# xiaohong-huang/RTK-Visual-Inertial-Navigation

Measured on AMD Instinct MI355X. Metric: gauss_newton_iterations_per_sec, higher is better.
Workload: dtype f64; 1 GPU; BASELINE cfg4: batch of 512 independent cfg3 windows (20 keyframes, 300 features, 3000 observations, 19 IMU factors, 10 satellites x 20 epochs carrier-phase+pseudorange, gauge prior) over the job, 8 dogleg iterations per solve; windows=512, windows_rank0=512

## Files before the change

rtk_visual_inertial_navigation_amd/csrc/swf_dev.h:

```cpp
#pragma once
#include <hip/hip_runtime.h>
#include <stdint.h>
#include "../../include/swf_types.h"

#define SWF_WAVE 64

struct WinRec {
    int x_base, x_n;
    int blk_base, n_blk;
    int loc_base, n_loc, n_e, n_red;
    long long S_base;
    long long Lt_base;
    int proj0, proj1;
    int lm0, lm1;
    int fr_base, nF;
    long long P_base;
    int gf0, gf1;
    int cl0, cl1;
    int pair0, pair1;
    int fsb0, fsb1;
    int tail_dim;
    int n_pose_blk;
    int lmb0, lmb1;
    int pch0, pch1;
// ... 9 lines not shown
    int status, iter, need_lin, reuse, eval_cand, lin_fail, invalid_run, nsucc, nunsucc;
    int chol_fail;
};

enum { GF_IMU = 1, GF_CP = 2, GF_PR = 3, GF_DOP = 4, GF_SP = 5, GF_PRIOR = 6, GF_SPR = 7, GF_SCP = 8, GF_FIX = 9, GF_IDP = 10,
       GF_PROJX = 11 };
struct GFac {
    int type, win, nres, nslot;
    int slot0;
    int roff;
    int data;
    int clique;
    int jld;
    int pad;
};

struct Clique {
    int win;
    int e_loc, d_e;
    int d_f;
    int fac0, fac1;
    int mem0, mem1;
    long long C_off;
    int v_off;
    int e_off;
    int is_static;
    int n_rows;
    int j_off, r_off;
    int pad0, pad1;
};
// ... 59 lines not shown
    const int* sch_c0; const int* sch_rec;
    const int* sch_km;
    const unsigned long long* lm_fmask;
    int n_fr;
    const int* fr_obs0; const int* fr_obs;
    const int* fr_red;
    int n_gf;
    const GFac* gf;
    const int* s_x; const int* s_loc; const int* s_ls; const int* s_joff; const int* s_ccol;
    double* g_r; double* g_J; double* g_cost; double* g_aux;
    const double* imu_pre; const double* cp_dat; const double* pr_dat; const double* dop_dat; const double* sp_w;
    const double* gx_dat;
    int n_imu; const int* imu_gf;
    int n_idp; const int* idp_gf;
    int n_sc;  const int* sc_gf;
    int n_prior; const int* prior_gf;
    int n_pch; const int* pch_q; const int* pch_r0; const int* prior_nch;
    double* pr_cpart; double* pr_apart;
    const int* prior_dim; const long long* prior_Joff; const int* prior_roff; const int* prior_x0off;
    const double* prior_J; const double* prior_r0; const double* prior_x0;
    const double* prior_Jt;
    const int* prior_colloc;
    const int* prior_colcc;
    const int* s_pcol; const int* s_pxo;
    int n_cl;
    const Clique* cl;
    const int* cl_fac; const int* cl_frow;
    const int* cm_loc; const int* cm_ls; const int* cm_col;
    double* C; double* cv_graw; double* cv_dgraw; double* cv_cs; double* cE;
    const int* cv_loc;
// ... 262 lines not shown
```

rtk_visual_inertial_navigation_amd/csrc/swf_engine.hip:

```cpp
#include <hip/hip_runtime.h>
#include <algorithm>
#include <array>
#include <chrono>
#include <cmath>
#include <cstdio>
#include <cstdlib>
#include <cstring>
#include <map>
#include <string>
#include <memory>
#include <thread>
#include <vector>
#include "../../include/swf_solver.h"
#include "swf_kernels2.h"
#include "swf_kernels3.h"
#include "swf_kernels4.h"
#include "swf_lambda.h"
#include "swf_features.h"

static thread_local std::string g_err;
static int fail(int code, const std::string& msg) { g_err = msg; return code; }
#define HIPCHK(x) do { hipError_t e_ = (x); if (e_ != hipSuccess) return fail(SWF_E_NODEVICE, std::string(#x) + ": " + hipGetErrorString(e_)); } while (0)

extern "C" const char* swf_last_error(void) { return g_err.c_str(); }
// ... 191 lines not shown
        if (aux) { (void)hipStreamSynchronize(aux); handle_cache().give(aux); }
        for (auto& e : ev_fork) handle_cache().give(e, false);
    }
    WinState* ws_primary = nullptr; WinState* ws_alt = nullptr; WinState* ws_alt2 = nullptr;
    bool no_decide_fuse = false;
    bool no_step_fuse = false;
    int n_pch_split = 0;
    bool no_spec = false;
    bool no_comp_fuse = false;
    bool lat_fuse = false;
    bool rr4_has15 = false, rr4_has16 = false;
    int rr_nmax = 256;
    bool L_full = false;
    int asm_programs = 0;
    int ls_qpb = 1, ls_var = 0, ls_kms = 8; bool ls_folded = false, s_direct = false;
    int timing = 0;
    swf_timing last{};
    std::vector<hipEvent_t> ev;
    std::vector<int> ev_kind;
    int ev_used = 0;
    int64_t jac_bytes = 0, proj_bytes = 0, chol_flops = 0, lm_schur_flops = 0, lm_schur_flops_sym = 0, lm_schur_mfma = 0;
    int last_mode = -1;
};

namespace {
struct Build {
    std::vector<WinRec> win;
    std::vector<int> blk_xoff, blk_loc, blk_gs, loc2x;
    std::vector<unsigned char> x_var;
    std::vector<int> p_win, p_xpose, p_xex, p_xlm, p_lpose, p_llm, p_fr, p_lm;
// ... 552 lines not shown
    std::vector<HostWin> hw(n);
    for (int i = 0; i < n; i++) {
        int rc = build_window(B, windows[i], i, hw[i]);
        if (rc != SWF_OK) return rc;
    }
    if (B.n_x > 0x7fffffffLL || B.n_loc > 0x7fffffffLL) return fail(SWF_E_UNSUPPORTED, "batch too large for 32-bit offsets");
    swf_batch* b = new swf_batch();
    b->device = current_device();
    b->stream = (hipStream_t)stream;
    { int dev = 0; hipDeviceProp_t pr; if (hipGetDevice(&dev) == hipSuccess && hipGetDeviceProperties(&pr, dev) == hipSuccess && pr.multiProcessorCount > 0) b->n_cu = pr.multiProcessorCount; }
    b->D.rr_nmax = b->rr_nmax;
    b->no_comp_fuse = getenv("SWF_NO_COMP_FUSE") != nullptr;
    b->no_spec = getenv("SWF_NO_SPEC_EVAL") != nullptr;
    b->no_step_fuse = getenv("SWF_NO_STEP_FUSE") != nullptr;
    b->no_decide_fuse = getenv("SWF_NO_DECIDE_FUSE") != nullptr;
    b->lat_fuse = n * 8 <= b->n_cu && !getenv("SWF_NO_LAT_FUSE");
    if ((n * 16 <= b->n_cu && !b->lat_fuse) || (2 * n >= b->n_cu && n <= b->n_cu)) {
        bool ok = (b->aux = handle_cache().stream()) != nullptr;
        for (int i = 0; i < 3 && ok; i++) ok = (b->ev_fork[i] = handle_cache().event(false)) != nullptr;
        if (!ok) { handle_cache().give(b->aux); b->aux = nullptr; }
    }
    b->win = B.win; b->hw = hw; b->max_tiles = B.max_tiles; b->max_prior_dim = B.max_prior_dim; b->jac_bytes = B.jac_bytes;
    b->proj_bytes = (int64_t)312 * (int64_t)B.p_win.size();
    for (size_t l = 0; l + 1 < B.lm_obs0.size() + 1 && l < B.lm_win.size(); l++) {
        int64_t k = (l + 1 < B.lm_obs0.size() ? B.lm_obs0[l + 1] : (int)B.p_win.size()) - B.lm_obs0[l];
        b->lm_schur_flops += 216 * k * k + 108 * k;
        b->lm_schur_flops_sym += 108 * k * (k - 1) + 162 * k;
    }
    for (auto& W : B.win) { b->chol_flops += (int64_t)W.n_red * W.n_red * W.n_red / 3; b->max_red = std::max(b->max_red, W.n_red); b->min_red = std::min(b->min_red, W.n_red); if (W.n_red > 224 && W.n_red <= 240) b->rr4_has15 = true; if (W.n_red > 240 && W.n_red <= 256) b->rr4_has16 = true; }
    DevBatch& D = b->D;
// ... 48 lines not shown
    PUT(p_lpose, B.p_lpose); PUT(p_llm, B.p_llm); PUT(p_fr, B.p_fr); PUT(p_lm, B.p_lm); PUT(p_uv, B.p_uv);
    D.n_lm = (int)B.lm_win.size();
    B.lm_obs0.push_back(D.n_proj);
    PUT(lm_win, B.lm_win); PUT(lm_obs0, B.lm_obs0); PUT(lm_loc, B.lm_loc); PUT(lm_col, B.lm_col); PUT(lm_fmask, B.lm_fmask);
    {
        const int force = getenv("SWF_LS_VARIANT") ? atoi(getenv("SWF_LS_VARIANT")) : 0;
        const int force_qpb = getenv("SWF_LS_QPB") ? atoi(getenv("SWF_LS_QPB")) : 0;
        int qpb = 1;
        while (qpb < GEMM_SPLIT && (long long)n * GEMM_SPLIT / (2 * qpb) >= 2LL * b->n_cu) qpb *= 2;
        if (2LL * n >= b->n_cu) qpb = GEMM_SPLIT;
        if (force_qpb >= 1 && force_qpb <= GEMM_SPLIT && (force_qpb & (force_qpb - 1)) == 0) qpb = force_qpb;
        b->ls_qpb = qpb;
        b->ls_var = (b->max_tiles <= 10 && force < 1) ? 0 : (b->max_tiles <= 36 && force < 2) ? 1 : (b->max_tiles <= 136 && force < 3) ? 2 : 3;
        b->ls_folded = qpb == GEMM_SPLIT && b->ls_var <= 1;
        b->s_direct = b->ls_folded;
    }
    {
        const int TW = b->ls_var <= 1 ? 2 : 1;
        const int NCW = b->ls_var <= 1 ? 8 : 12, TPW = b->ls_var == 0 ? 2 : b->ls_var == 1 ? 5 : 6;
        const int n_launch = std::max(1, (b->max_tiles + NCW * TPW - 1) / (NCW * TPW));
        b->ls_kms = n_launch * NCW;
        std::vector<int> c0, rec, km;
        std::vector<std::vector<unsigned>> task_tiles;
        for (auto& W : B.win) {
            const int m = 6 * W.nF, nt = (m + 15) / 16, ntl = nt * (nt + 1) / 2;
            auto tile_rows = [&](unsigned long long fm) {
                unsigned t = 0;
                for (int f = 0; f < W.nF && f < 64; f++) if ((fm >> f) & 1ULL) { t |= 1u << ((6 * f) / 16); t |= 1u << ((6 * f + 5) / 16); }
                return t;
            };
// ... 58 lines not shown
            int* r = rec.data() + (size_t)8 * k;
            r[0] = B.fsb_win[(size_t)k]; r[1] = B.fsb_obs0[(size_t)k]; r[2] = B.fsb_obs0[(size_t)k + 1] - B.fsb_obs0[(size_t)k];
            r[3] = B.fsb_foff0[(size_t)k]; r[4] = B.fsb_out0[(size_t)k]; r[5] = B.win[(size_t)r[0]].nF;
        }
        PUT(fsb_rec, rec);
    }
    PUT(fsb_perm, B.fsb_perm); PUT(fsb_foff, B.fsb_foff);
    rc |= P.zeros((size_t)B.fs_tot * FS_VAL, &D.fs_part);
    rc |= P.zeros((size_t)std::max<long long>(B.n_loc, 1), &D.jsc);
    D.n_gf = (int)B.gf.size();
    PUT(gf, B.gf);
    PUT(s_x, B.s_x); PUT(s_loc, B.s_loc); PUT(s_ls, B.s_ls); PUT(s_joff, B.s_joff); PUT(s_ccol, B.s_ccol);
    PUT(imu_pre, B.imu_pre); PUT(cp_dat, B.cp_dat); PUT(pr_dat, B.pr_dat); PUT(dop_dat, B.dop_dat); PUT(sp_w, B.sp_w); PUT(gx_dat, B.gx_dat);
    D.n_imu = (int)B.imu_gf.size(); D.n_sc = (int)B.sc_gf.size(); D.n_prior = (int)B.prior_gf.size();
    PUT(imu_gf, B.imu_gf); PUT(sc_gf, B.sc_gf); PUT(prior_gf, B.prior_gf); D.n_idp = (int)B.idp_gf.size(); PUT(idp_gf, B.idp_gf);
    PUT(prior_dim, B.prior_dim); PUT(prior_Joff, B.prior_Joff); PUT(prior_roff, B.prior_roff); PUT(prior_x0off, B.prior_x0off);
    {
        std::vector<double> Jt(B.prior_J.size());
        for (size_t k = 0; k < B.prior_dim.size(); k++) {
            const size_t n = (size_t)B.prior_dim[k]; const double* J = B.prior_J.data() + B.prior_Joff[k]; double* T = Jt.data() + B.prior_Joff[k];
            for (size_t r = 0; r < n; r++) for (size_t c = 0; c < n; c++) T[c * n + r] = J[r * n + c];
        }
        PUT(prior_Jt, Jt);
        std::vector<int> cl(B.prior_r0.size(), -1), cc(B.prior_r0.size(), -1), pcol(B.s_ls.size(), 0), pxo(B.s_ls.size(), 0);
        for (const GFac& G : B.gf) {
            if (G.type != GF_PRIOR) continue;
            int col = 0, xo = 0;
            for (int t = 0; t < G.nslot; t++) {
                int l = B.s_ls[G.slot0 + t], lo = B.s_loc[G.slot0 + t], mc = B.s_ccol[G.slot0 + t];
                pcol[G.slot0 + t] = col; pxo[G.slot0 + t] = xo;
// ... 479 lines not shown
            if (imu_fused) hipLaunchKernelGGL((k_eval_ps<true, true, true>), dim3(S.e[3]), dim3(256), 0, st, D, S);
            else hipLaunchKernelGGL((k_eval_ps<true, true>), dim3(S.e[2]), dim3(256), 0, st, D, S);
        }
        if (D.n_idp) hipLaunchKernelGGL(k_eval_idp<true>, GRID(D.n_idp, 128), dim3(128), 0, st, D);
        if (D.n_prior && b->max_prior_dim > PRIOR_LDS_DIM) { Bracket t(*this, SWF_K_EVAL_PRIOR); hipLaunchKernelGGL(k_eval_prior<true>, dim3(D.n_pch), dim3(256), (2 * b->max_prior_dim + 16) * sizeof(double), st, D); }
        if (fork) (void)hipEventRecord(b->ev_fork[1], st);
        if (D.n_imu && !imu_fused) { Bracket t(*this, SWF_K_EVAL_IMU, sa); hipLaunchKernelGGL(k_eval_imu<true>, GRID(D.n_imu, IMU_FPB), dim3(IMU_FPB * IMU_LPF), 0, sa, D); }
    }
    void lin_elim(int write_S) {
        DevBatch& D = b->D;
        bool clq_fused = false;
        if (comp_fused) {
            Bracket t(*this, SWF_K_CLIQUE_ELIM);
            if (D.n_clc[3]) {
                hipLaunchKernelGGL(k_clique_big2, dim3(D.n_clc[3] + D.n_clc[2]), dim3(CB_NT), 0, st, D, O);
                if (D.n_clc[4]) hipLaunchKernelGGL(k_clique_tall, dim3(D.n_clc[4]), dim3(256), 0, st, D, O);
            } else if (D.n_clc[4] + D.n_clc[2]) hipLaunchKernelGGL(k_clique_tall2, dim3(D.n_clc[4] + D.n_clc[2]), dim3(256), 0, st, D, O);
        } else if (D.n_lm) {
            Bracket t(*this, write_S ? SWF_K_LM_SCHUR : SWF_K_LM_ELIM);
            lm_qpb = b->ls_qpb; lm_folded = b->ls_folded;
            if (!write_S) {
                dim3 grid(D.n_win, GEMM_SPLIT / lm_qpb);
                hipLaunchKernelGGL((k_lm_schur<8, 2, 2, 80, false>), grid, dim3(256), 0, st, D, O, lm_qpb, 0, 0, 0);
            } else {
                const int crow = D.n_win > 0 ? (D.n_clc[2] + D.n_win - 1) / D.n_win : 0;
                clq_fused = clq_fuse_ok();
                lm_launch(0, st, clq_fused ? crow : 0);
                lm_next = ls_tiles_per_launch();
            }
        }
        {
            hipStream_t sa = b->aux ? b->aux : st;
            if (b->aux) (void)hipStreamWaitEvent(b->aux, b->ev_fork[1], 0);
            auto cstream = [&](int cls) { return (b->aux && !b->clc_imu[cls]) ? st : sa; };
            if (comp_fused) {
                for (; lm_next < b->max_tiles; lm_next += ls_tiles_per_launch()) { Bracket t(*this, SWF_K_LM_SCHUR, sa); lm_launch(lm_next, sa); }
            } else {
            if (D.n_clc[1]) { Bracket t(*this, SWF_K_CLIQUE_ELIM, cstream(1)); hipLaunchKernelGGL((k_clique_elim<32, 48, 9, 1>), dim3(D.n_clc[1]), dim3(64), 0, cstream(1), D, O); }
            if (D.n_clc[0]) { Bracket t(*this, SWF_K_CLIQUE_ELIM, cstream(0)); hipLaunchKernelGGL((k_clique_elim<48, 32, 1, 0>), dim3(D.n_clc[0]), dim3(64), 0, cstream(0), D, O); }
            if (D.n_clc[2] && !clq_fused) {
                Bracket t(*this, SWF_K_CLIQUE_ELIM, cstream(2));
                if (b->lat_fuse) hipLaunchKernelGGL(k_clique_elim4, dim3(D.n_clc[2]), dim3(256), 0, cstream(2), D, O);
                else hipLaunchKernelGGL((k_clique_elim<64, 64, 9, 2>), dim3(D.n_clc[2]), dim3(64), 0, cstream(2), D, O);
            }
            if (D.n_clc[3]) { Bracket t(*this, SWF_K_CLIQUE_ELIM, cstream(3)); hipLaunchKernelGGL(k_clique_big, dim3(D.n_clc[3]), dim3(CB_NT), 0, cstream(3), D, O); }
            if (D.n_clc[4]) { Bracket t(*this, SWF_K_CLIQUE_ELIM, cstream(4)); hipLaunchKernelGGL(k_clique_tall, dim3(D.n_clc[4]), dim3(256), 0, cstream(4), D, O); }
            if (write_S && D.n_lm) {
                for (; lm_next < b->max_tiles; lm_next += ls_tiles_per_launch()) { Bracket t(*this, SWF_K_LM_SCHUR, sa); lm_launch(lm_next, sa); }
            }
            }
            if (b->aux) (void)hipEventRecord(b->ev_fork[2], b->aux);
        }
        if (b->n_pch_split) hipLaunchKernelGGL(k_prior_graw, dim3(D.n_pch), dim3(256), 0, st, D);
        if (b->aux) (void)hipStreamWaitEvent(st, b->ev_fork[2], 0);
        if (D.n_pd) {
            Bracket t(*this, SWF_K_ASSEMBLE);
            const int nbS = write_S ? nb((size_t)D.as_max_ne, 256) : 0, nbV = nb((size_t)D.as_max_nv, 256);
            hipLaunchKernelGGL(k_assemble_flat, dim3(nbS + nbV, D.n_win), dim3(256), 0, st, D, O, write_S, nbS);
        }
    }
    void reduced() {
// ... 871 lines not shown
```

rtk_visual_inertial_navigation_amd/csrc/swf_kernels.h:

```cpp
#pragma once
#include "swf_dev.h"

struct DevOpt {
    int max_iter, step_mode, strategy, jacobi;
    double r0, max_r, min_r, min_rel_dec, ftol, gtol, ptol, min_mu, max_mu, mu_inc, min_diag, max_diag;
};



__device__ __forceinline__ double damp_diag(const DevOpt& O, double d, double* jsc_slot, bool first) {
    if (!O.jacobi) return clampd(d, O.min_diag, O.max_diag);
    double q;
    if (first) { double r = 1.0 + sqrt(d > 0.0 ? d : 0.0); q = r * r; *jsc_slot = q; }
    else q = *jsc_slot;
    return clampd(d / q, O.min_diag, O.max_diag) * q;
}

template <bool JAC> __device__ __forceinline__ bool eval_gate(const DevBatch& B, const WinState& s) { return B.spec == 2 ? true : (JAC && !B.spec) ? s.need_lin != 0 : s.eval_cand != 0; }
template <bool JAC> __device__ __forceinline__ const double* eval_src(const DevBatch& B) { return (JAC && !B.spec) ? B.x : B.xc; }

#define CLIGHT_D 299792458.0
#define OMGE_D 7.2921151467E-5

template <bool JAC, bool STORE>
// ... 707 lines not shown
            if (jo < 0) continue;
            int l = B.s_ls[G.slot0 + t], lo = B.s_loc[G.slot0 + t];
            const double* col0 = B.g_J + jo + k;
            for (int j0 = 0; j0 < l; j0 += 9) {
                double c[9], v[9];
#pragma unroll
                for (int j = 0; j < 9; j++) { bool ok = j0 + j < l; c[j] = ok ? col0[(j0 + j) * G.jld] : 0.0; v[j] = ok ? vec_at<MODE>(B, O, lo + j0 + j) : 0.0; }
#pragma unroll
                for (int j = 0; j < 9; j++) if (j0 + j < l) a += c[j] * v[j];
            }
        }
    }
    return a;
}
template <int MODE>
__device__ __forceinline__ double gf_row_term(const DevBatch& B, const GFac& G, int k, double a) {
    return MODE == 0 ? a * a : a * (B.g_r[G.roff + k] + a / 2.0);
}
template <int MODE>
__device__ __forceinline__ void d_jtimes_scalar(const DevBatch& B, const DevOpt& O, int bid) {
    int q = bid * blockDim.x + threadIdx.x;
    if (q >= B.n_sc) return;
    int f = B.sc_gf[q];
    const GFac& G = B.gf[f];
    const WinState& s = B.ws[G.win];
    if (MODE == 0 ? !s.need_lin : !s.eval_cand) return;
    double a = 0;
    for (int k = 0; k < G.nres; k++) a += gf_row_term<MODE>(B, G, k, gf_row_dot<MODE>(B, O, G, k));
    B.g_aux[f] = a;
}
template <int MODE>
__device__ __forceinline__ void d_jtimes_imu(const DevBatch& B, const DevOpt& O, int bid) {
    int q = (bid * blockDim.x + threadIdx.x) >> 4, sub = threadIdx.x & 15;
    bool valid = q < B.n_imu;
    int f = B.imu_gf[valid ? q : B.n_imu - 1];
    const GFac& G = B.gf[f];
    const WinState& s = B.ws[G.win];
    bool act = valid && (MODE == 0 ? s.need_lin : s.eval_cand);
    double part = 0;
    if (act && sub < 15) part = gf_row_term<MODE>(B, G, sub, gf_row_dot<MODE>(B, O, G, sub));
    part = grp16_sum(part);
    if (act && sub == 0) B.g_aux[f] = part;
}
#define PRB_MAX 512
template <int MODE>
__device__ __forceinline__ void d_jtimes_prior(const DevBatch& B, const DevOpt& O, int blk, double* sv, int* sl, double* sw) {
    const int tid = threadIdx.x;
    if (blk >= B.n_pch) return;
    const int q = B.pch_q[blk], k_lo = B.pch_r0[blk];
    const bool chunked = B.prior_nch[q] > 1;
    int f = B.prior_gf[q];
    const GFac& G = B.gf[f];
    const WinState& s = B.ws[G.win];
    if (MODE == 0 ? !s.need_lin : !s.eval_cand) return;
    const int n = G.nres;
    const bool staged = n <= PRB_MAX;
    const int* cl = B.prior_colloc + B.prior_roff[G.data];
// ... 44 lines not shown
}

#include "swf_lmschur.h"

#define CLQ_MAXD 64
#define CLQ_MAXR 64
#ifdef SWF_PROFILE_CLQ
__device__ unsigned long long g_clq_stamps[16];
#ifndef SWF_PROFILE_CLQ_IDX
#define SWF_PROFILE_CLQ_IDX 0
#endif
#define QST(i) do { if (cidx_ == SWF_PROFILE_CLQ_IDX && threadIdx.x == 0) { unsigned long long t_ = __builtin_amdgcn_s_memtime(); g_clq_stamps[i] += t_ - tq_; tq_ = t_; } } while (0)
#else
#define QST(i)
#endif
template <int MAXR, int MAXD, int MAXE, int CLS, int PF = 24, int NW = 1, int UK = 4>
__device__ __forceinline__ void d_clique_elim(const DevBatch& B, const DevOpt& O, const int cidx_) {
    constexpr int LD = MAXD + 1, NT = 64 * NW;
    __shared__ double Jc[MAXR][LD];
    __shared__ double Me[MAXE][MAXD];
    __shared__ double T[MAXE][MAXD];
    __shared__ double Ei[MAXE][MAXE];
    __shared__ double rv[MAXR];
    __shared__ double Eg[MAXE];
    __shared__ double gcs[NW > 1 ? MAXD : 1];
    __shared__ int bad_sh;
#ifdef SWF_PROFILE_CLQ
    unsigned long long tq_ = __builtin_amdgcn_s_memtime();
    if (cidx_ == SWF_PROFILE_CLQ_IDX && threadIdx.x == 0) for (int i = 0; i < 16; i++) g_clq_stamps[i] = 0;
#endif
    if (cidx_ >= B.n_clc[CLS]) return;
// ... 13 lines not shown
        for (int base = 0; base < tot; base += PF * NT) {
            double v[PF];
#pragma unroll
            for (int u = 0; u < PF; u++) { int e = base + u * NT + tid; v[u] = e < tot ? gJ[e] : 0.0; }
#pragma unroll
            for (int u = 0; u < PF; u++) {
                int e = base + u * NT + tid;
                int col = (int)((e + 0.5f) * rd);
                col += (e - col * nrow >= nrow) ? 1 : 0; col -= (e - col * nrow < 0) ? 1 : 0;
                if (e < tot) Jc[e - col * nrow][col] = v[u];
            }
        }
    }
    __syncthreads();
    QST(1);
    double me[MAXE], gc = 0, mcc = 0;
#pragma unroll
    for (int a2 = 0; a2 < MAXE; a2++) me[a2] = 0;
    {
        int c = lane < d ? lane : 0;
        if (NW == 1) {
#pragma unroll UK
            for (int k = 0; k < nrow; k++) {
                double x = Jc[k][c];
                gc += x * rv[k]; mcc += x * x;
#pragma unroll
                for (int a2 = 0; a2 < MAXE; a2++) me[a2] += Jc[k][a2] * x;
            }
        } else {
            constexpr int RPW = (MAXE + NW - 1) / NW;
#pragma unroll UK
            for (int k = 0; k < nrow; k++) {
                double x = Jc[k][c];
                if (wq == 0) { gc += x * rv[k]; mcc += x * x; }
#pragma unroll
                for (int u = 0; u < RPW; u++) { int a2 = wq + u * NW; if (a2 < MAXE) me[u] += Jc[k][a2] * x; }
            }
        }
    }
    if (lane < d) {
        if (NW == 1) {
#pragma unroll
            for (int a2 = 0; a2 < MAXE; a2++) Me[a2][lane] = a2 < de ? me[a2] : 0.0;
        } else {
            constexpr int RPW = (MAXE + NW - 1) / NW;
#pragma unroll
            for (int u = 0; u < RPW; u++) { int a2 = wq + u * NW; if (a2 < MAXE) Me[a2][lane] = a2 < de ? me[u] : 0.0; }
        }
        if (wq == 0) {
            if (NW > 1) gcs[lane] = gc;
            if (lane < de) { B.g[C.e_loc + lane] = gc; B.diag[C.e_loc + lane] = mcc; B.vc[C.e_loc + lane] = gc / clampd(mcc, O.min_diag, O.max_diag); }
            else { B.cv_graw[C.v_off + lane - de] = gc; B.cv_dgraw[C.v_off + lane - de] = mcc; }
        }
    }
    __syncthreads();
    QST(2);
    if (de > 0) {
        if (wq == 0) {
            double row[2 * MAXE];
#pragma unroll
            for (int j = 0; j < MAXE; j++) {
                double v = (lane < de && j < de) ? Me[lane][j] : 0.0;
                if (j == lane) v += s.mu * (lane < de ? damp_diag(O, v, B.jsc + C.e_loc + lane, s.iter == 0) : clampd(v, O.min_diag, O.max_diag));
                row[j] = v; row[MAXE + j] = (j == lane) ? 1.0 : 0.0;
            }
            bool bad = false;
#pragma unroll
            for (int k = 0; k < MAXE; k++) {
                if (k < de) {
// ... 112 lines not shown
            }
#pragma unroll
            for (int u = 0; u < 2; u++) {
                if (!on[u]) continue;
                int i = i0[u], j = j0[u];
                bool i1ok = i + 1 < df, j1ok = j + 1 < df;
                Cm[i * df + j] = m[u][0]; Cm[j * df + i] = m[u][0];
                if (i1ok) { Cm[(i + 1) * df + j] = m[u][2]; Cm[j * df + i + 1] = m[u][2]; }
                if (!diag[u] && j1ok) { Cm[i * df + j + 1] = m[u][1]; Cm[(j + 1) * df + i] = m[u][1]; }
                if (i1ok && j1ok) { Cm[(i + 1) * df + j + 1] = m[u][3]; Cm[(j + 1) * df + i + 1] = m[u][3]; }
            }
        }
    }
    QST(5);
}
template <int MAXR, int MAXD, int MAXE, int CLS>
__global__ void __launch_bounds__(64) k_clique_elim(DevBatch B, DevOpt O) { d_clique_elim<MAXR, MAXD, MAXE, CLS>(B, O, (int)blockIdx.x); }
__global__ void __launch_bounds__(256) k_clique_elim4(DevBatch B, DevOpt O) { d_clique_elim<64, 64, 9, 2, 8, 4>(B, O, (int)blockIdx.x); }
#define CLQ_TALLR 96
__global__ void __launch_bounds__(256) k_clique_tall(DevBatch B, DevOpt O) { d_clique_elim<CLQ_TALLR, 64, 9, 4, 8, 4>(B, O, (int)blockIdx.x); }

template <int NCW, int TPW, int TW, int LDR>
__global__ void __launch_bounds__(LS_NT(NCW, TW)) k_lm_clique(DevBatch B, DevOpt O, int qpb, int lp, int kms, int s_direct, int n_parts) {
    if ((int)blockIdx.y < n_parts) d_lm_schur<NCW, TPW, TW, LDR, true>(B, O, qpb, lp, kms, s_direct, (int)blockIdx.x, (int)blockIdx.y);
    else {
        constexpr int CLQ_NW = 4;
        static_assert(CLQ_NW * 64 == 256 && LS_NT(NCW, TW) >= CLQ_NW * 64, "k_lm_clique: the clique rows keep exactly the waves d_clique_elim<..., NW> synchronises");
        if (threadIdx.x >= CLQ_NW * 64) return;
        d_clique_elim<64, 64, 9, 2, 8, 4, CLQ_NW>(B, O, ((int)blockIdx.y - n_parts) * (int)gridDim.x + (int)blockIdx.x);
    }
}

#define CB_MAXD 768
#define CB_MAXED 1536
#define CB_LDS_J 12288
// ... 272 lines not shown
```

rtk_visual_inertial_navigation_amd/csrc/swf_lmschur.h:

```cpp
#pragma once
typedef double double4_t __attribute__((ext_vector_type(4)));
#define GEMM_SPLIT 16
#ifdef SWF_PROFILE_GEMM
__device__ unsigned long long g_gemm_stamps[16];
#define GSTAMP_ACC(i, t0) do { if (bx_ == 0 && by_ == 0 && (threadIdx.x & 63) == 0) g_gemm_stamps[i] += __builtin_amdgcn_s_memtime() - (t0); } while (0)
#define GNOW() __builtin_amdgcn_s_memtime()
#else
#define GSTAMP_ACC(i, t0)
#define GNOW() 0ULL
#endif
#define LS_NB 4
#define LS_NT(NCW, TW) ((LS_NB * (TW) + (NCW)) * 64)
#define LS_MAXF 64
#define LS_SPIN_MAX (1 << 22)
struct LsRec { int L, loc, o0, o1, col, info; };
struct LsDat { double jl[6], rr[2]; int f; };
__device__ __forceinline__ void ls_wait(const unsigned* flag, unsigned target, WinState& s) {
    asm volatile("" ::: "memory");
    for (int spin = 0; ; spin++) {
        unsigned v = __hip_atomic_load(flag, __ATOMIC_RELAXED, __HIP_MEMORY_SCOPE_WORKGROUP);
        if ((int)((unsigned)__builtin_amdgcn_readfirstlane((int)v) - target) >= 0) break;
        if (spin >= LS_SPIN_MAX) { s.lin_fail = 1; break; }
        __builtin_amdgcn_s_sleep(1);
    }
    asm volatile("" ::: "memory");
}
__device__ __forceinline__ void ls_signal(unsigned* flag) {
    asm volatile("" ::: "memory");
    if ((threadIdx.x & 63) == 0) __hip_atomic_fetch_add(flag, 1u, __ATOMIC_RELAXED, __HIP_MEMORY_SCOPE_WORKGROUP);
    asm volatile("" ::: "memory");
}
template <int NCW, int TPW, int TW, int LDR, bool GEMM>
__device__ __forceinline__ void d_lm_schur(const DevBatch& B, const DevOpt& O, int qpb, int lp, int kms, int s_direct, const int bx_, const int by_) {
    constexpr int NPW = GEMM ? LS_NB * TW : 4;
    constexpr int NCOL = 12 * TW, NG = TW;
    constexpr int PANEL = NCOL * LDR;
    constexpr int KSB = 4 * LDR * 8;
    static_assert(!GEMM || LS_NB * PANEL < 0xffff, "panel offsets are kept in 16 bits");
    __shared__ double Zp[GEMM ? LS_NB * PANEL + LS_NB * NCOL : 1];
    __shared__ unsigned flg[2 * LS_NB];
    __shared__ int freds[LS_MAXF];
    double* const hb = Zp + (GEMM ? LS_NB * PANEL : 0);
    const int tile_base = lp * NCW * TPW;
    int w = bx_, sp0 = by_ * qpb;
    const bool outs = tile_base == 0;
    WinState& s = B.ws[w];
    if (!s.need_lin) return;
    const WinRec& W = B.win[w];
// ... 230 lines not shown
            h00 += FMA2(b[0], b[0], b[3], b[3]); h10 += FMA2(b[1], b[0], b[4], b[3]); h20 += FMA2(b[2], b[0], b[5], b[3]);
            h11 += FMA2(b[1], b[1], b[4], b[4]); h21 += FMA2(b[2], b[1], b[5], b[4]); h22 += FMA2(b[2], b[2], b[5], b[5]);
            g0 += FMA2(b[0], d2.rr[0], b[3], d2.rr[1]); g1 += FMA2(b[1], d2.rr[0], b[4], d2.rr[1]); g2 += FMA2(b[2], d2.rr[0], b[5], d2.rr[1]);
        }
        h00 = grp16_sum(h00); h10 = grp16_sum(h10); h20 = grp16_sum(h20); h11 = grp16_sum(h11); h21 = grp16_sum(h21); h22 = grp16_sum(h22);
        g0 = grp16_sum(g0); g1 = grp16_sum(g1); g2 = grp16_sum(g2);
        if (wv == 0) GSTAMP_ACC(0, tg);
        tg = GNOW();
        const bool lead = act && sub == 0;
        if (lead && outs) {
            B.g[loc] = g0; B.g[loc + 1] = g1; B.g[loc + 2] = g2;
            B.diag[loc] = h00; B.diag[loc + 1] = h11; B.diag[loc + 2] = h22;
            B.vc[loc] = g0 * rcp_nr(clampd(h00, O.min_diag, O.max_diag)); B.vc[loc + 1] = g1 * rcp_nr(clampd(h11, O.min_diag, O.max_diag)); B.vc[loc + 2] = g2 * rcp_nr(clampd(h22, O.min_diag, O.max_diag));
        }
        double i00 = 0, i11 = 0, i22 = 0, i10 = 0, i20 = 0, i21 = 0;
        if (act) {
            const bool jfirst = s.iter == 0;
            h00 = __builtin_fma(mu, damp_diag(O, h00, B.jsc + loc, jfirst), h00);
            h11 = __builtin_fma(mu, damp_diag(O, h11, B.jsc + loc + 1, jfirst), h11);
            h22 = __builtin_fma(mu, damp_diag(O, h22, B.jsc + loc + 2, jfirst), h22);
            i00 = rsqrt_nr(h00);
            double l10 = h10 * i00, l20 = h20 * i00;
            double d11 = __builtin_fma(-l10, l10, h11);
            i11 = rsqrt_nr(d11);
            double l21 = __builtin_fma(-l20, l10, h21) * i11;
            double d22 = __builtin_fma(-l21, l21, __builtin_fma(-l20, l20, h22));
            i22 = rsqrt_nr(d22);
            bool bad = !(h00 > 0.0) || !(d11 > 0.0) || !(d22 > 0.0);
            if (bad) { if (lead && outs) s.lin_fail = 1; i00 = i11 = i22 = 0.0; }
            i10 = -l10 * i00 * i11;
            i21 = -l21 * i11 * i22;
// ... 77 lines not shown
    if (!GEMM || gemm) {
        LsRec rc = load_rec(task), rn = load_rec(task + tstep), rnn;
        LsDat da, db;
        load_dat(rc, da, 0);
        while (task < t1) {
            run_task(rc, da, rn, db, rnn);
            rc = rn; rn = rnn;
            if (task >= t1) break;
            run_task(rc, db, rn, da, rnn);
            rc = rn; rn = rnn;
        }
    }
    if (wv == 0) GSTAMP_ACC(6, tall);
    }
}
template <int NCW, int TPW, int TW, int LDR, bool GEMM>
__global__ void __launch_bounds__(GEMM ? LS_NT(NCW, TW) : 256) k_lm_schur(DevBatch B, DevOpt O, int qpb, int lp, int kms, int s_direct) {
    d_lm_schur<NCW, TPW, TW, LDR, GEMM>(B, O, qpb, lp, kms, s_direct, (int)blockIdx.x, (int)blockIdx.y);
}
```

Baseline: 670,500 iterations/s.

## Add gradient-only final elimination and precomputed Jacobian-times records for scalar/IMU factors

When the Schur complement is not written (the final elimination pass), the landmark Schur and clique-elimination kernels now run gradient-only variants. These skip the damped 3x3 inverse and the E-block products, and the clique kernel exits extra waves early. Scalar and IMU Jacobian-times kernels now read a compact 96-byte per-factor record holding slot offsets instead of chasing the GFac and slot arrays. They also compute unconditionally and gate only the store, which avoids divergence. This assumes the final pass needs only g, diag and vc, so correctness depends on downstream code not consuming the skipped outputs.

Result: faster. 688,800 iterations/s (median of 6 runs) (+2.7%).

```diff
diff --git a/rtk_visual_inertial_navigation_amd/csrc/swf_dev.h b/rtk_visual_inertial_navigation_amd/csrc/swf_dev.h
--- a/rtk_visual_inertial_navigation_amd/csrc/swf_dev.h
+++ b/rtk_visual_inertial_navigation_amd/csrc/swf_dev.h
@@ -47,6 +47,17 @@
     int jld;
     int pad;
 };
+
+#define JT_MAXSLOT 5
+struct alignas(16) JtRec {
+    int win, nres, jld, nslot;
+    int roff, f, pad0, pad1;
+    int joff[JT_MAXSLOT];
+    int loc[JT_MAXSLOT];
+    int ls[JT_MAXSLOT];
+    int pad2;
+};
+static_assert(sizeof(JtRec) == 96, "JtRec: six 16-byte loads");
 
 struct Clique {
     int win;
@@ -136,6 +147,7 @@
     int n_imu; const int* imu_gf;
     int n_idp; const int* idp_gf;
     int n_sc;  const int* sc_gf;
+    const JtRec* sc_jt; const JtRec* imu_jt;
     int n_prior; const int* prior_gf;
     int n_pch; const int* pch_q; const int* pch_r0; const int* prior_nch;
     double* pr_cpart; double* pr_apart;
diff --git a/rtk_visual_inertial_navigation_amd/csrc/swf_engine.hip b/rtk_visual_inertial_navigation_amd/csrc/swf_engine.hip
--- a/rtk_visual_inertial_navigation_amd/csrc/swf_engine.hip
+++ b/rtk_visual_inertial_navigation_amd/csrc/swf_engine.hip
@@ -229,6 +229,8 @@
     bool L_full = false;
     int asm_programs = 0;
     int ls_qpb = 1, ls_var = 0, ls_kms = 8; bool ls_folded = false, s_direct = false;
+    bool full_final = false;
+    int ls_gqpb = 4;
     int timing = 0;
     swf_timing last{};
     std::vector<hipEvent_t> ev;
@@ -811,6 +813,7 @@
     b->no_spec = getenv("SWF_NO_SPEC_EVAL") != nullptr;
     b->no_step_fuse = getenv("SWF_NO_STEP_FUSE") != nullptr;
     b->no_decide_fuse = getenv("SWF_NO_DECIDE_FUSE") != nullptr;
+    b->full_final = getenv("SWF_FULL_FINAL_ELIM") != nullptr;
     b->lat_fuse = n * 8 <= b->n_cu && !getenv("SWF_NO_LAT_FUSE");
     if ((n * 16 <= b->n_cu && !b->lat_fuse) || (2 * n >= b->n_cu && n <= b->n_cu)) {
         bool ok = (b->aux = handle_cache().stream()) != nullptr;
@@ -889,6 +892,9 @@
         b->ls_var = (b->max_tiles <= 10 && force < 1) ? 0 : (b->max_tiles <= 36 && force < 2) ? 1 : (b->max_tiles <= 136 && force < 3) ? 2 : 3;
         b->ls_folded = qpb == GEMM_SPLIT && b->ls_var <= 1;
         b->s_direct = b->ls_folded;
+        const int force_gqpb = getenv("SWF_LS_GRAD_QPB") ? atoi(getenv("SWF_LS_GRAD_QPB")) : 0;
+        b->ls_gqpb = std::min(qpb, LS_GRAD_QPB);
+        if (force_gqpb >= 1 && force_gqpb <= GEMM_SPLIT && (force_gqpb & (force_gqpb - 1)) == 0) b->ls_gqpb = force_gqpb;
     }
     {
         const int TW = b->ls_var <= 1 ? 2 : 1;
@@ -977,6 +983,27 @@
     PUT(imu_pre, B.imu_pre); PUT(cp_dat, B.cp_dat); PUT(pr_dat, B.pr_dat); PUT(dop_dat, B.dop_dat); PUT(sp_w, B.sp_w); PUT(gx_dat, B.gx_dat);
     D.n_imu = (int)B.imu_gf.size(); D.n_sc = (int)B.sc_gf.size(); D.n_prior = (int)B.prior_gf.size();
     PUT(imu_gf, B.imu_gf); PUT(sc_gf, B.sc_gf); PUT(prior_gf, B.prior_gf); D.n_idp = (int)B.idp_gf.size(); PUT(idp_gf, B.idp_gf);
+    {
+        bool fits = true;
+        auto jt_recs = [&](const std::vector<int>& list) {
+            std::vector<JtRec> out(list.size());
+            for (size_t q = 0; q < list.size(); q++) {
+                const GFac& G = B.gf[(size_t)list[q]];
+                JtRec& r = out[q];
+                r = JtRec{};
+                r.win = G.win; r.nres = G.nres; r.jld = G.jld; r.nslot = G.nslot; r.roff = G.roff; r.f = list[q];
+                if (G.nslot > JT_MAXSLOT) { fits = false; continue; }
+                for (int t = 0; t < JT_MAXSLOT; t++) {
+                    const bool has = t < G.nslot;
+                    r.joff[t] = has ? B.s_joff[(size_t)G.slot0 + t] : -1; r.loc[t] = has ? B.s_loc[(size_t)G.slot0 + t] : 0; r.ls[t] = has ? B.s_ls[(size_t)G.slot0 + t] : 0;
+                }
+            }
+            return out;
+        };
+        const std::vector<JtRec> sj = jt_recs(B.sc_gf), ij = jt_recs(B.imu_gf);
+        if (!fits) { P.release(); delete b; return fail(SWF_E_UNSUPPORTED, "scalar / IMU factor with more than JT_MAXSLOT parameter blocks"); }
+        PUT(sc_jt, sj); PUT(imu_jt, ij);
+    }
     PUT(prior_dim, B.prior_dim); PUT(prior_Joff, B.prior_Joff); PUT(prior_roff, B.prior_roff); PUT(prior_x0off, B.prior_x0off);
     {
         std::vector<double> Jt(B.prior_J.size());
@@ -1486,12 +1513,15 @@
             Bracket t(*this, SWF_K_CLIQUE_ELIM);
             if (D.n_clc[3]) {
                 hipLaunchKernelGGL(k_clique_big2, dim3(D.n_clc[3] + D.n_clc[2]), dim3(CB_NT), 0, st, D, O);
-                if (D.n_clc[4]) hipLaunchKernelGGL(k_clique_tall, dim3(D.n_clc[4]), dim3(256), 0, st, D, O);
+                if (D.n_clc[4]) hipLaunchKernelGGL(k_clique_tall<false>, dim3(D.n_clc[4]), dim3(256), 0, st, D, O);
             } else if (D.n_clc[4] + D.n_clc[2]) hipLaunchKernelGGL(k_clique_tall2, dim3(D.n_clc[4] + D.n_clc[2]), dim3(256), 0, st, D, O);
         } else if (D.n_lm) {
             Bracket t(*this, write_S ? SWF_K_LM_SCHUR : SWF_K_LM_ELIM);
             lm_qpb = b->ls_qpb; lm_folded = b->ls_folded;
-            if (!write_S) {
+            if (!write_S && !b->full_final) {
+                dim3 grid(D.n_win, GEMM_SPLIT / b->ls_gqpb);
+                hipLaunchKernelGGL((k_lm_schur<8, 2, 2, 80, false, true>), grid, dim3(256), 0, st, D, O, b->ls_gqpb, 0, 0, 0);
+            } else if (!write_S) {
                 dim3 grid(D.n_win, GEMM_SPLIT / lm_qpb);
                 hipLaunchKernelGGL((k_lm_schur<8, 2, 2, 80, false>), grid, dim3(256), 0, st, D, O, lm_qpb, 0, 0, 0);
             } else {
@@ -1508,15 +1538,32 @@
             if (comp_fused) {
                 for (; lm_next < b->max_tiles; lm_next += ls_tiles_per_launch()) { Bracket t(*this, SWF_K_LM_SCHUR, sa); lm_launch(lm_next, sa); }
             } else {
-            if (D.n_clc[1]) { Bracket t(*this, SWF_K_CLIQUE_ELIM, cstream(1)); hipLaunchKernelGGL((k_clique_elim<32, 48, 9, 1>), dim3(D.n_clc[1]), dim3(64), 0, cstream(1), D, O); }
-            if (D.n_clc[0]) { Bracket t(*this, SWF_K_CLIQUE_ELIM, cstream(0)); hipLaunchKernelGGL((k_clique_elim<48, 32, 1, 0>), dim3(D.n_clc[0]), dim3(64), 0, cstream(0), D, O); }
+            const bool grad = !write_S && !b->full_final;
+            if (D.n_clc[1]) {
+                Bracket t(*this, SWF_K_CLIQUE_ELIM, cstream(1));
+                if (grad) hipLaunchKernelGGL((k_clique_elim<32, 48, 9, 1, true>), dim3(D.n_clc[1]), dim3(64), 0, cstream(1), D, O);
+                else hipLaunchKernelGGL((k_clique_elim<32, 48, 9, 1>), dim3(D.n_clc[1]), dim3(64), 0, cstream(1), D, O);
+            }
+            if (D.n_clc[0]) {
+                Bracket t(*this, SWF_K_CLIQUE_ELIM, cstream(0));
+                if (grad) hipLaunchKernelGGL((k_clique_elim<48, 32, 1, 0, true>), dim3(D.n_clc[0]), dim3(64), 0, cstream(0), D, O);
+                else hipLaunchKernelGGL((k_clique_elim<48, 32, 1, 0>), dim3(D.n_clc[0]), dim3(64), 0, cstream(0), D, O);
+            }
             if (D.n_clc[2] && !clq_fused) {
                 Bracket t(*this, SWF_K_CLIQUE_ELIM, cstream(2));
-                if (b->lat_fuse) hipLaunchKernelGGL(k_clique_elim4, dim3(D.n_clc[2]), dim3(256), 0, cstream(2), D, O);
+                if (b->lat_fuse) {
+                    if (grad) hipLaunchKernelGGL(k_clique_elim4<true>, dim3(D.n_clc[2]), dim3(256), 0, cstream(2), D, O);
+                    else hipLaunchKernelGGL(k_clique_elim4<false>, dim3(D.n_clc[2]), dim3(256), 0, cstream(2), D, O);
+                }
+                else if (grad) hipLaunchKernelGGL((k_clique_elim<64, 64, 9, 2, true>), dim3(D.n_clc[2]), dim3(64), 0, cstream(2), D, O);
                 else hipLaunchKernelGGL((k_clique_elim<64, 64, 9, 2>), dim3(D.n_clc[2]), dim3(64), 0, cstream(2), D, O);
             }
             if (D.n_clc[3]) { Bracket t(*this, SWF_K_CLIQUE_ELIM, cstream(3)); hipLaunchKernelGGL(k_clique_big, dim3(D.n_clc[3]), dim3(CB_NT), 0, cstream(3), D, O); }
-            if (D.n_clc[4]) { Bracket t(*this, SWF_K_CLIQUE_ELIM, cstream(4)); hipLaunchKernelGGL(k_clique_tall, dim3(D.n_clc[4]), dim3(256), 0, cstream(4), D, O); }
+            if (D.n_clc[4]) {
+                Bracket t(*this, SWF_K_CLIQUE_ELIM, cstream(4));
+                if (grad) hipLaunchKernelGGL(k_clique_tall<true>, dim3(D.n_clc[4]), dim3(256), 0, cstream(4), D, O);
+                else hipLaunchKernelGGL(k_clique_tall<false>, dim3(D.n_clc[4]), dim3(256), 0, cstream(4), D, O);
+            }
             if (write_S && D.n_lm) {
                 for (; lm_next < b->max_tiles; lm_next += ls_tiles_per_launch()) { Bracket t(*this, SWF_K_LM_SCHUR, sa); lm_launch(lm_next, sa); }
             }
diff --git a/rtk_visual_inertial_navigation_amd/csrc/swf_kernels.h b/rtk_visual_inertial_navigation_amd/csrc/swf_kernels.h
--- a/rtk_visual_inertial_navigation_amd/csrc/swf_kernels.h
+++ b/rtk_visual_inertial_navigation_amd/csrc/swf_kernels.h
@@ -745,33 +745,58 @@
     return a;
 }
 template <int MODE>
-__device__ __forceinline__ double gf_row_term(const DevBatch& B, const GFac& G, int k, double a) {
-    return MODE == 0 ? a * a : a * (B.g_r[G.roff + k] + a / 2.0);
+__device__ __forceinline__ double gf_row_term(const DevBatch& B, int roff, int k, double a) {
+    return MODE == 0 ? a * a : a * (B.g_r[roff + k] + a / 2.0);
+}
+template <int MODE>
+__device__ __forceinline__ double gf_row_term(const DevBatch& B, const GFac& G, int k, double a) { return gf_row_term<MODE>(B, G.roff, k, a); }
+template <int MODE, int CH = 16>
+__device__ __forceinline__ double jt_row_dot(const DevBatch& B, const DevOpt& O, const JtRec& R, int k) {
+    int e[JT_MAXSLOT], ncol = 0;
+#pragma unroll
+    for (int t = 0; t < JT_MAXSLOT; t++) { ncol += (t < R.nslot && R.joff[t] >= 0) ? R.ls[t] : 0; e[t] = ncol; }
+    double a = 0;
+    for (int u0 = 0; u0 < ncol; u0 += CH) {
+        double c[CH], v[CH];
+#pragma unroll
+        for (int j = 0; j < CH; j++) {
+            const int u = u0 + j;
+            int jo = R.joff[0], lo = R.loc[0], st = 0;
+#pragma unroll
+            for (int t = 1; t < JT_MAXSLOT; t++) if (u >= e[t - 1]) { jo = R.joff[t]; lo = R.loc[t]; st = e[t - 1]; }
+            const bool ok = u < ncol;
+            c[j] = B.g_J[ok ? jo + (u - st) * R.jld + k : 0];
+            v[j] = vec_at<MODE>(B, O, ok ? lo + (u - st) : 0);
+        }
+#pragma unroll
+        for (int j = 0; j < CH; j++) if (u0 + j < ncol) a += c[j] * v[j];
+    }
+    return a;
 }
 template <int MODE>
 __device__ __forceinline__ void d_jtimes_scalar(const DevBatch& B, const DevOpt& O, int bid) {
     int q = bid * blockDim.x + threadIdx.x;
-    if (q >= B.n_sc) return;
-    int f = B.sc_gf[q];
-    const GFac& G = B.gf[f];
-    const WinState& s = B.ws[G.win];
-    if (MODE == 0 ? !s.need_lin : !s.eval_cand) return;
+    const bool valid = q < B.n_sc;
+    const JtRec R = B.sc_jt[valid ? q : B.n_sc - 1];
+    const WinState& s = B.ws[R.win];
+    const int gate = MODE == 0 ? s.need_lin : s.eval_cand;
     double a = 0;
-    for (int k = 0; k < G.nres; k++) a += gf_row_term<MODE>(B, G, k, gf_row_dot<MODE>(B, O, G, k));
-    B.g_aux[f] = a;
+    for (int k = 0; k < R.nres; k++) a += gf_row_term<MODE>(B, R.roff, k, jt_row_dot<MODE>(B, O, R, k));
+    if (valid && gate) B.g_aux[R.f] = a;
 }
 template <int MODE>
 __device__ __forceinline__ void d_jtimes_imu(const DevBatch& B, const DevOpt& O, int bid) {
     int q = (bid * blockDim.x + threadIdx.x) >> 4, sub = threadIdx.x & 15;
-    bool valid = q < B.n_imu;
-    int f = B.imu_gf[valid ? q : B.n_imu - 1];
-    const GFac& G = B.gf[f];
-    const WinState& s = B.ws[G.win];
-    bool act = valid && (MODE == 0 ? s.need_lin : s.eval_cand);
-    double part = 0;
-    if (act && sub < 15) part = gf_row_term<MODE>(B, G, sub, gf_row_dot<MODE>(B, O, G, sub));
+    const bool valid = q < B.n_imu;
+    const JtRec R = B.imu_jt[valid ? q : B.n_imu - 1];
+    const WinState& s = B.ws[R.win];
+    const int gate = MODE == 0 ? s.need_lin : s.eval_cand;
+    const int k = sub < 15 ? sub : 14;
+    double part = gf_row_term<MODE>(B, R.roff, k, jt_row_dot<MODE>(B, O, R, k));
+    const bool act = valid && gate;
+    if (!(act && sub < 15)) part = 0;
     part = grp16_sum(part);
-    if (act && sub == 0) B.g_aux[f] = part;
+    if (act && sub == 0) B.g_aux[R.f] = part;
 }
 #define PRB_MAX 512
 template <int MODE>
@@ -846,7 +871,7 @@
 #else
 #define QST(i)
 #endif
-template <int MAXR, int MAXD, int MAXE, int CLS, int PF = 24, int NW = 1, int UK = 4>
+template <int MAXR, int MAXD, int MAXE, int CLS, int PF = 24, int NW = 1, int UK = 4, bool GRAD = false>
 __device__ __forceinline__ void d_clique_elim(const DevBatch& B, const DevOpt& O, const int cidx_) {
     constexpr int LD = MAXD + 1, NT = 64 * NW;
     __shared__ double Jc[MAXR][LD];
@@ -890,6 +915,7 @@
     }
     __syncthreads();
     QST(1);
+    if (GRAD && wq != 0) return;
     double me[MAXE], gc = 0, mcc = 0;
 #pragma unroll
     for (int a2 = 0; a2 < MAXE; a2++) me[a2] = 0;
@@ -900,8 +926,10 @@
             for (int k = 0; k < nrow; k++) {
                 double x = Jc[k][c];
                 gc += x * rv[k]; mcc += x * x;
+                if (!GRAD) {
 #pragma unroll
                 for (int a2 = 0; a2 < MAXE; a2++) me[a2] += Jc[k][a2] * x;
+                }
             }
         } else {
             constexpr int RPW = (MAXE + NW - 1) / NW;
@@ -909,26 +937,29 @@
             for (int k = 0; k < nrow; k++) {
                 double x = Jc[k][c];
                 if (wq == 0) { gc += x * rv[k]; mcc += x * x; }
+                if (!GRAD) {
 #pragma unroll
                 for (int u = 0; u < RPW; u++) { int a2 = wq + u * NW; if (a2 < MAXE) me[u] += Jc[k][a2] * x; }
+                }
             }
         }
     }
     if (lane < d) {
-        if (NW == 1) {
+        if (!GRAD && NW == 1) {
 #pragma unroll
             for (int a2 = 0; a2 < MAXE; a2++) Me[a2][lane] = a2 < de ? me[a2] : 0.0;
-        } else {
+        } else if (!GRAD) {
             constexpr int RPW = (MAXE + NW - 1) / NW;
 #pragma unroll
             for (int u = 0; u < RPW; u++) { int a2 = wq + u * NW; if (a2 < MAXE) Me[a2][lane] = a2 < de ? me[u] : 0.0; }
         }
         if (wq == 0) {
-            if (NW > 1) gcs[lane] = gc;
+            if (NW > 1 && !GRAD) gcs[lane] = gc;
             if (lane < de) { B.g[C.e_loc + lane] = gc; B.diag[C.e_loc + lane] = mcc; B.vc[C.e_loc + lane] = gc / clampd(mcc, O.min_diag, O.max_diag); }
             else { B.cv_graw[C.v_off + lane - de] = gc; B.cv_dgraw[C.v_off + lane - de] = mcc; }
         }
     }
+    if (GRAD) return;
     __syncthreads();
     QST(2);
     if (de > 0) {
@@ -1071,11 +1102,13 @@
     }
     QST(5);
 }
-template <int MAXR, int MAXD, int MAXE, int CLS>
-__global__ void __launch_bounds__(64) k_clique_elim(DevBatch B, DevOpt O) { d_clique_elim<MAXR, MAXD, MAXE, CLS>(B, O, (int)blockIdx.x); }
-__global__ void __launch_bounds__(256) k_clique_elim4(DevBatch B, DevOpt O) { d_clique_elim<64, 64, 9, 2, 8, 4>(B, O, (int)blockIdx.x); }
+template <int MAXR, int MAXD, int MAXE, int CLS, bool GRAD = false>
+__global__ void __launch_bounds__(64) k_clique_elim(DevBatch B, DevOpt O) { d_clique_elim<MAXR, MAXD, MAXE, CLS, 24, 1, 4, GRAD>(B, O, (int)blockIdx.x); }
+template <bool GRAD = false>
+__global__ void __launch_bounds__(256) k_clique_elim4(DevBatch B, DevOpt O) { d_clique_elim<64, 64, 9, 2, 8, 4, 4, GRAD>(B, O, (int)blockIdx.x); }
 #define CLQ_TALLR 96
-__global__ void __launch_bounds__(256) k_clique_tall(DevBatch B, DevOpt O) { d_clique_elim<CLQ_TALLR, 64, 9, 4, 8, 4>(B, O, (int)blockIdx.x); }
+template <bool GRAD = false>
+__global__ void __launch_bounds__(256) k_clique_tall(DevBatch B, DevOpt O) { d_clique_elim<CLQ_TALLR, 64, 9, 4, 8, 4, 4, GRAD>(B, O, (int)blockIdx.x); }
 
 template <int NCW, int TPW, int TW, int LDR>
 __global__ void __launch_bounds__(LS_NT(NCW, TW)) k_lm_clique(DevBatch B, DevOpt O, int qpb, int lp, int kms, int s_direct, int n_parts) {
diff --git a/rtk_visual_inertial_navigation_amd/csrc/swf_lmschur.h b/rtk_visual_inertial_navigation_amd/csrc/swf_lmschur.h
--- a/rtk_visual_inertial_navigation_amd/csrc/swf_lmschur.h
+++ b/rtk_visual_inertial_navigation_amd/csrc/swf_lmschur.h
@@ -9,6 +9,7 @@
 #define GSTAMP_ACC(i, t0)
 #define GNOW() 0ULL
 #endif
+#define LS_GRAD_QPB 4
 #define LS_NB 4
 #define LS_NT(NCW, TW) ((LS_NB * (TW) + (NCW)) * 64)
 #define LS_MAXF 64
@@ -30,8 +31,9 @@
     if ((threadIdx.x & 63) == 0) __hip_atomic_fetch_add(flag, 1u, __ATOMIC_RELAXED, __HIP_MEMORY_SCOPE_WORKGROUP);
     asm volatile("" ::: "memory");
 }
-template <int NCW, int TPW, int TW, int LDR, bool GEMM>
+template <int NCW, int TPW, int TW, int LDR, bool GEMM, bool GRAD = false>
 __device__ __forceinline__ void d_lm_schur(const DevBatch& B, const DevOpt& O, int qpb, int lp, int kms, int s_direct, const int bx_, const int by_) {
+    static_assert(!(GEMM && GRAD), "the gradient-only form has no product");
     constexpr int NPW = GEMM ? LS_NB * TW : 4;
     constexpr int NCOL = 12 * TW, NG = TW;
     constexpr int PANEL = NCOL * LDR;
@@ -292,7 +294,7 @@
             B.vc[loc] = g0 * rcp_nr(clampd(h00, O.min_diag, O.max_diag)); B.vc[loc + 1] = g1 * rcp_nr(clampd(h11, O.min_diag, O.max_diag)); B.vc[loc + 2] = g2 * rcp_nr(clampd(h22, O.min_diag, O.max_diag));
         }
         double i00 = 0, i11 = 0, i22 = 0, i10 = 0, i20 = 0, i21 = 0;
-        if (act) {
+        if (act && !GRAD) {
             const bool jfirst = s.iter == 0;
             h00 = __builtin_fma(mu, damp_diag(O, h00, B.jsc + loc, jfirst), h00);
             h11 = __builtin_fma(mu, damp_diag(O, h11, B.jsc + loc + 1, jfirst), h11);
@@ -400,7 +402,7 @@
     if (wv == 0) GSTAMP_ACC(6, tall);
     }
 }
-template <int NCW, int TPW, int TW, int LDR, bool GEMM>
+template <int NCW, int TPW, int TW, int LDR, bool GEMM, bool GRAD = false>
 __global__ void __launch_bounds__(GEMM ? LS_NT(NCW, TW) : 256) k_lm_schur(DevBatch B, DevOpt O, int qpb, int lp, int kms, int s_direct) {
-    d_lm_schur<NCW, TPW, TW, LDR, GEMM>(B, O, qpb, lp, kms, s_direct, (int)blockIdx.x, (int)blockIdx.y);
+    d_lm_schur<NCW, TPW, TW, LDR, GEMM, GRAD>(B, O, qpb, lp, kms, s_direct, (int)blockIdx.x, (int)blockIdx.y);
 }
```
